# craston/object_detection_cib

Hardware: AMD Instinct MI355X
Metric: images/sec YOLOv5s 640px train (higher is better)
Workload: dtype bf16; 1 GPU; yv5s coco-zipf-like synthetic, 640px, bf16 storage/fp32 accumulate, batch 64/GPU, fwd+assign+loss+bwd+SGD, targets 4-30 boxes/img; global_batch=64, parallelism=dp1, launch=hipGraph replay, collectives=none, launcher=none, attempt=0

## Files before the change

### object_detection_cib_amd/csrc/bn_act.hip

```cpp
#include "kodhip_common.h"
#include <stdlib.h>

namespace {

__device__ __forceinline__ double wave_sum_partials(const float* p, int T, int lane) {
  double a0 = 0.0, a1 = 0.0, a2 = 0.0, a3 = 0.0;
  const int T4 = ((reinterpret_cast<uintptr_t>(p) & 15) == 0) ? (T & ~3) : 0;
#pragma unroll 4
  for (int t = lane * 4; t < T4; t += 256) {
    f32x4 v = *reinterpret_cast<const f32x4*>(p + t);
    a0 += (double)v[0]; a1 += (double)v[1]; a2 += (double)v[2]; a3 += (double)v[3];
  }
  for (int t = T4 + lane; t < T; t += 64) a0 += (double)p[t];
  return wave_sum_d((a0 + a1) + (a2 + a3));
}

__device__ __forceinline__ void wave_sum_partials2(const float* p, const float* q, int T, int lane, double& sp, double& sq) {
  const bool al = ((reinterpret_cast<uintptr_t>(p) | reinterpret_cast<uintptr_t>(q)) & 15) == 0;
  if (!al || T > 4 * 256) {
    sp = wave_sum_partials(p, T, lane);
    sq = wave_sum_partials(q, T, lane);
    return;
  }
  const int T4 = T & ~3;
  const int t0 = lane * 4, t1 = t0 + 256 * 1, t2 = t0 + 256 * 2, t3 = t0 + 256 * 3;
  const f32x4 z = {0.f, 0.f, 0.f, 0.f};
  f32x4 pv[4], qv[4];
  const int ts[4] = {t0, t1, t2, t3};
#pragma unroll
  for (int i = 0; i < 4; ++i) {
    pv[i] = ts[i] < T4 ? *reinterpret_cast<const f32x4*>(p + ts[i]) : z;
    qv[i] = ts[i] < T4 ? *reinterpret_cast<const f32x4*>(q + ts[i]) : z;
  }
  float pt = 0.f, qt = 0.f;
  const bool tail = T4 + lane < T;
  if (tail) { pt = p[T4 + lane]; qt = q[T4 + lane]; }
  double a[4] = {0.0, 0.0, 0.0, 0.0}, b[4] = {0.0, 0.0, 0.0, 0.0};
#pragma unroll
  for (int i = 0; i < 4; ++i) {
    if (ts[i] < T4) {
#pragma unroll
      for (int e = 0; e < 4; ++e) { a[e] += (double)pv[i][e]; b[e] += (double)qv[i][e]; }
    }
  }
  if (tail) { a[0] += (double)pt; b[0] += (double)qt; }
  sp = wave_sum_d((a[0] + a[1]) + (a[2] + a[3]));
  sq = wave_sum_d((b[0] + b[1]) + (b[2] + b[3]));
}

__device__ __forceinline__ void peer_allreduce2(const KodPeerView& pv, unsigned int slot, int idx0, int idx1, int lane,
                                                double& s0, double& s1) {
  const unsigned int seq = *pv.seq;
  const unsigned long long b0 = __shfl((unsigned long long)__double_as_longlong(s0), 0, 64);
  const unsigned long long b1 = __shfl((unsigned long long)__double_as_longlong(s1), 0, 64);
  const int g = lane & 3;
  const unsigned long long gi = (unsigned long long)slot + 2ull * (unsigned long long)(g < 2 ? idx0 : idx1) + (g & 1);
  if (lane < 4) {
    const unsigned long long bits = g < 2 ? b0 : b1;
    const unsigned int payload = (unsigned int)((g & 1) ? (bits >> 32) : bits);
    __hip_atomic_store(pv.peers[pv.rank] + gi, ((unsigned long long)seq << 32) | payload, __ATOMIC_RELAXED, __HIP_MEMORY_SCOPE_SYSTEM);
  }
  unsigned int got = 0;
  bool bad = false;
  const int r = lane >> 2;
  if (r < pv.world) got = (unsigned int)kod_peer_poll(pv, pv.peers[r] + gi, seq, bad);
  double t0 = 0.0, t1 = 0.0;
  for (int q = 0; q < pv.world; ++q) {
    const unsigned long long lo0 = __shfl(got, 4 * q + 0, 64), hi0 = __shfl(got, 4 * q + 1, 64);
    const unsigned long long lo1 = __shfl(got, 4 * q + 2, 64), hi1 = __shfl(got, 4 * q + 3, 64);
    t0 += __longlong_as_double((long long)((hi0 << 32) | lo0));
    t1 += __longlong_as_double((long long)((hi1 << 32) | lo1));
  }
  if (__ballot(bad) != 0ull) t0 = t1 = __longlong_as_double(0x7ff8000000000000ll);
  s0 = t0; s1 = t1;
}

__global__ void bn_reduce_partials_kernel(const float* part, double* sums, int C, int T) {
  int idx = blockIdx.x * (blockDim.x >> 6) + (threadIdx.x >> 6);
  if (idx >= 2 * C) return;
  int lane = threadIdx.x & 63;
  double s = wave_sum_partials(part + (size_t)idx * T, T, lane);
  if (lane == 0) sums[idx] = s;
}

__global__ void bn_finalize_kernel(const double* sums, double count, const float* gamma, const float* beta,
                                   float* running_mean, float* running_var, float momentum, float eps,
                                   float* scale, float* shift, float* mean_out, float* rstd_out, int C,
                                   int update_running) {
  int c = blockIdx.x * blockDim.x + threadIdx.x;
  if (c >= C) return;
  double mean = sums[c] / count;
  double var = sums[C + c] / count - mean * mean;
  if (var < 0.0) var = 0.0;
  float rstd = (float)(1.0 / sqrt(var + (double)eps));
  float g = gamma[c], b = beta[c];
  float sc = g * rstd;
  scale[c] = sc;
  shift[c] = b - (float)mean * sc;
  mean_out[c] = (float)mean;
  rstd_out[c] = rstd;
  if (update_running) {
    double unbiased = count > 1.0 ? var * count / (count - 1.0) : var;
    running_mean[c] = (1.f - momentum) * running_mean[c] + momentum * (float)mean;
    running_var[c] = (1.f - momentum) * running_var[c] + momentum * (float)unbiased;
  }
}

template <bool PEER>
__global__ void bn_finalize_fused_kernel(const float* part, int T, double count, const float* gamma,
                                         const float* beta, float* running_mean, float* running_var,
                                         float momentum, float eps, float* scale, float* shift, float* mean_out,
                                         float* rstd_out, int C, int update_running, KodPeerView pv, unsigned int slot) {
  int c = blockIdx.x * (blockDim.x >> 6) + (threadIdx.x >> 6);
  if (c >= C) return;
  int lane = threadIdx.x & 63;
  const float* p0 = part + (size_t)c * T;
  const float* p1 = part + (size_t)(C + c) * T;
  const float g = gamma[c], b = beta[c];
  const float rm0 = update_running ? running_mean[c] : 0.f, rv0 = update_running ? running_var[c] : 0.f;
  double s0, s1;
  wave_sum_partials2(p0, p1, T, lane, s0, s1);
  if constexpr (PEER) peer_allreduce2(pv, slot, c, C + c, lane, s0, s1);
  if (lane != 0) return;
  double mean = s0 / count;
  double var = s1 / count - mean * mean;
  if (var < 0.0) var = 0.0;
  float rstd = (float)(1.0 / sqrt(var + (double)eps));
  float sc = g * rstd;
  scale[c] = sc;
  shift[c] = b - (float)mean * sc;
  mean_out[c] = (float)mean;
  rstd_out[c] = rstd;
  if (update_running) {
    double unbiased = count > 1.0 ? var * count / (count - 1.0) : var;
    running_mean[c] = (1.f - momentum) * rm0 + momentum * (float)mean;
    running_var[c] = (1.f - momentum) * rv0 + momentum * (float)unbiased;
  }
}

template <bool PEER = false, bool EVAL = false>
__device__ __forceinline__ void bn_bwd_coeffs_channel(const float* part, int T, double count, const float* gamma,
                                                      const float* mean, const float* rstd, float* dgamma, float* dbeta,
                                                      float* coef, int C, int raw_moment, int c, int lane,
                                                      const KodPeerView* pv = nullptr, unsigned int slot = 0) {
  const float* p0 = part + (size_t)c * T;
  const float* p1 = part + (size_t)(C + c) * T;
  const float g_ = gamma[c], rs_ = rstd[c], mu_ = mean[c];
  double s0, s1;
  wave_sum_partials2(p0, p1, T, lane, s0, s1);
  if (raw_moment) s1 = (double)rs_ * (s1 - (double)mu_ * s0);
  if (lane == 0) {
    dbeta[c] = (float)s0;
    dgamma[c] = (float)s1;
  }
  if constexpr (EVAL) {
    static_assert(!PEER, "an eval-mode unit exchanges nothing");
    if (lane == 0) {
      coef[c] = (float)((double)g_ * (double)rs_);
      coef[C + c] = 0.f;
      coef[2 * C + c] = 0.f;
    }
    return;
  }
  if constexpr (PEER) peer_allreduce2(*pv, slot, c, C + c, lane, s0, s1);
  if (lane != 0) return;
  double g = g_, rs = rs_, mu = mu_;
  double S0 = s0 / count, S1 = s1 / count;
  coef[c] = (float)(g * rs);
  coef[C + c] = (float)(-g * rs * rs * S1);
  coef[2 * C + c] = (float)(-g * rs * S0 + g * rs * rs * mu * S1);
}

__global__ void bn_bwd_coeffs_fused_kernel(const float* part, int T, double count, const float* gamma,
                                           const float* mean, const float* rstd, float* dgamma, float* dbeta,
                                           float* coef, int C, int raw_moment) {
  int c = blockIdx.x * (blockDim.x >> 6) + (threadIdx.x >> 6);
  if (c >= C) return;
  bn_bwd_coeffs_channel(part, T, count, gamma, mean, rstd, dgamma, dbeta, coef, C, raw_moment, c, threadIdx.x & 63);
}

__global__ void bn_bwd_coeffs_peer_kernel(const float* part, int T, double count, const float* gamma,
                                          const float* mean, const float* rstd, float* dgamma, float* dbeta,
                                          float* coef, int C, int raw_moment, KodPeerView pv, unsigned int slot) {
  int c = blockIdx.x * (blockDim.x >> 6) + (threadIdx.x >> 6);
  if (c >= C) return;
  bn_bwd_coeffs_channel<true>(part, T, count, gamma, mean, rstd, dgamma, dbeta, coef, C, raw_moment, c, threadIdx.x & 63, &pv, slot);
}

struct CoefJob { const float* part; int T; double count; const float* gamma; const float* mean; const float* rstd;
                 float* dgamma; float* dbeta; float* coef; int C; int raw_moment; };
__global__ void bn_bwd_coeffs_fused2_kernel(CoefJob j0, CoefJob j1) {
  const CoefJob& j = blockIdx.y == 0 ? j0 : j1;
  int c = blockIdx.x * (blockDim.x >> 6) + (threadIdx.x >> 6);
  if (c >= j.C) return;
  bn_bwd_coeffs_channel(j.part, j.T, j.count, j.gamma, j.mean, j.rstd, j.dgamma, j.dbeta, j.coef, j.C, j.raw_moment, c,
                        threadIdx.x & 63);
}

__global__ void bn_bwd_coeffs_eval_kernel(const float* part, int T, const float* gamma, const float* mean,
                                          const float* rstd, float* dgamma, float* dbeta, float* coef, int C,
                                          int raw_moment) {
  int c = blockIdx.x * (blockDim.x >> 6) + (threadIdx.x >> 6);
  if (c >= C) return;
  bn_bwd_coeffs_channel<false, true>(part, T, 1.0, gamma, mean, rstd, dgamma, dbeta, coef, C, raw_moment, c,
                                     threadIdx.x & 63);
}

__global__ void bn_bwd_coeffs_mode2_kernel(CoefJob j0, CoefJob j1, int eval0, int eval1) {
  const CoefJob& j = blockIdx.y == 0 ? j0 : j1;
  int c = blockIdx.x * (blockDim.x >> 6) + (threadIdx.x >> 6);
  if (c >= j.C) return;
  if (blockIdx.y == 0 ? eval0 : eval1)
    bn_bwd_coeffs_channel<false, true>(j.part, j.T, j.count, j.gamma, j.mean, j.rstd, j.dgamma, j.dbeta, j.coef, j.C,
                                       j.raw_moment, c, threadIdx.x & 63);
  else
    bn_bwd_coeffs_channel(j.part, j.T, j.count, j.gamma, j.mean, j.rstd, j.dgamma, j.dbeta, j.coef, j.C, j.raw_moment,
                          c, threadIdx.x & 63);
}

struct BnEvalDesc {
  const float* gamma; const float* beta; const float* running_mean; const float* running_var;
  float* aff; float* coef; long long C; long long reserved;
};

__global__ __launch_bounds__(256) void bn_eval_constants_kernel(const BnEvalDesc* desc, float eps) {
  const BnEvalDesc d = desc[blockIdx.x];
  const int C = (int)d.C;
  for (int c = threadIdx.x; c < C; c += blockDim.x) {
    const float g = d.gamma[c], b = d.beta[c], rm = d.running_mean[c];
    const float rstd = (float)(1.0 / sqrt((double)d.running_var[c] + (double)eps));
    const float sc = g * rstd;
    d.aff[c] = sc;
    d.aff[C + c] = b - rm * sc;
    d.aff[2 * C + c] = rm;
    d.aff[3 * C + c] = rstd;
    if (d.coef != nullptr) {
      d.coef[c] = (float)((double)g * (double)rstd);
      d.coef[C + c] = 0.f;
      d.coef[2 * C + c] = 0.f;
    }
  }
}

constexpr int U = 4;

template <int ACT, int U, bool LDSK, int MAXT>
__global__ __launch_bounds__(MAXT) void bn_silu_apply_kernel(const bf16_t* y, int ldy, const float* scale, const float* shift,
                                     const bf16_t* res, int ldr, int rcoff,
                                     bf16_t* out, int ldo, int ocoff, long M, int C, int rows_per_block_iter, float slope) {
  extern __shared__ float kconst[];
// ... 488 lines not shown
```

### object_detection_cib_amd/csrc/kodhip_common.h

```cpp
#pragma once
#include <hip/hip_runtime.h>
#include <stdint.h>
#include <stdio.h>
#include <type_traits>

typedef __bf16 bf16_t;
typedef __bf16 bf16x8 __attribute__((ext_vector_type(8)));
typedef __bf16 bf16x4 __attribute__((ext_vector_type(4)));
typedef float f32x16 __attribute__((ext_vector_type(16)));
typedef float f32x4 __attribute__((ext_vector_type(4)));
typedef short s16x4 __attribute__((ext_vector_type(4)));
typedef unsigned int u32x4 __attribute__((ext_vector_type(4)));

#define KOD_OK 0
#define KOD_EARG (-1)

extern "C" void kodhip_set_error(const char* fmt, ...);

#define KOD_CHECK_ARG(cond, ...)                 \
  do {                                           \
    if (!(cond)) {                               \
      kodhip_set_error(__VA_ARGS__);             \
      return KOD_EARG;                           \
    }                                            \
  } while (0)

#define KOD_LAUNCH_CHECK(name)                                             \
  do {                                                                     \
    hipError_t e__ = hipGetLastError();                                    \
    if (e__ != hipSuccess) {                                               \
      kodhip_set_error("%s: %s", name, hipGetErrorString(e__));            \
      return (int)e__;                                                     \
    }                                                                      \
  } while (0)

#ifndef KOD_NO_NT
template <typename V> __device__ __forceinline__ V kod_load_once(const void* p) { return __builtin_nontemporal_load(reinterpret_cast<const V*>(p)); }
#else
template <typename V> __device__ __forceinline__ V kod_load_once(const void* p) { return *reinterpret_cast<const V*>(p); }
#endif

__device__ __forceinline__ float bf2f(bf16_t v) { return (float)v; }
__device__ __forceinline__ bf16_t f2bf(float v) { return (bf16_t)v; }

__device__ __forceinline__ float silu_f(float z) { return z / (1.0f + __expf(-z)); }
__device__ __forceinline__ float sigmoid_f(float z) { return 1.0f / (1.0f + __expf(-z)); }

#define KOD_NEG_LOG2E (-1.4426950408889634f)
__device__ __forceinline__ float kod_sigmoid_l2(float zl) {
  return __builtin_amdgcn_rcpf(1.0f + __builtin_amdgcn_exp2f(zl));
}
__device__ __forceinline__ float kod_silu_bwd(float g, float z, float sg) {
  const float t = __builtin_fmaf(-z, sg, z);
  return g * __builtin_fmaf(sg, t, sg);
}

enum { ACT_SILU = 0, ACT_RELU = 1, ACT_LEAKY = 2, ACT_HARDSWISH = 3, ACT_IDENTITY = 4 };
template <int ACT> __device__ __forceinline__ float kod_act(float z, float slope) {
  if (ACT == ACT_SILU) return z * kod_sigmoid_l2(KOD_NEG_LOG2E * z);
  if (ACT == ACT_RELU) return z > 0.f ? z : 0.f;
  if (ACT == ACT_LEAKY) return z > 0.f ? z : z * slope;
  if (ACT == ACT_HARDSWISH) return z * fminf(fmaxf(z + 3.f, 0.f), 6.f) / 6.f;
  return z;
}
template <int ACT> __device__ __forceinline__ float kod_act_bwd(float g, float z, float slope) {
  if (ACT == ACT_SILU) return kod_silu_bwd(g, z, kod_sigmoid_l2(KOD_NEG_LOG2E * z));
  if (ACT == ACT_RELU) return z > 0.f ? g : 0.f;
  if (ACT == ACT_LEAKY) return z > 0.f ? g : g * slope;
  if (ACT == ACT_HARDSWISH) return z <= -3.f ? 0.f : (z < 3.f ? g * ((z / 3.f) + 0.5f) : g);
  return g;
}
template <bool SILU = true, typename F> __host__ __device__ __forceinline__ void kod_with_act(int act, F&& f) {
  if constexpr (SILU) {
    if (act == ACT_SILU) return f(std::integral_constant<int, ACT_SILU>{});
  }
  if (act == ACT_RELU) f(std::integral_constant<int, ACT_RELU>{});
  else if (act == ACT_LEAKY) f(std::integral_constant<int, ACT_LEAKY>{});
  else if (act == ACT_HARDSWISH) f(std::integral_constant<int, ACT_HARDSWISH>{});
  else f(std::integral_constant<int, ACT_IDENTITY>{});
}

__device__ __forceinline__ float wave_sum(float v) {
#pragma unroll
  for (int o = 32; o > 0; o >>= 1) v += __shfl_xor(v, o, 64);
  return v;
}
__device__ __forceinline__ double wave_sum_d(double v) {
#pragma unroll
  for (int o = 32; o > 0; o >>= 1) v += __shfl_xor(v, o, 64);
  return v;
}

#define KOD_PEER_MAX 8
struct KodPeerView {
  unsigned long long* peers[KOD_PEER_MAX];
  int world, rank;
  const unsigned int* seq;
  int* timeout_flag;
  int* host_flag;
  long max_spins;
};

__device__ __forceinline__ unsigned long long kod_peer_poll(const KodPeerView& pv, const unsigned long long* src,
                                                            unsigned int seq, bool& bad) {
  const int raised = __hip_atomic_load(pv.timeout_flag, __ATOMIC_RELAXED, __HIP_MEMORY_SCOPE_AGENT);
  unsigned long long v = 0;
  long spins = 0;
  for (;;) {
    v = __hip_atomic_load(src, __ATOMIC_RELAXED, __HIP_MEMORY_SCOPE_SYSTEM);
    const unsigned int tag = (unsigned int)(v >> 32);
    if (tag == seq) break;
    int why = 0;
    if ((int)(tag - seq) > 0) why = 2;
    else if (raised) why = raised;
    else if (++spins > pv.max_spins) why = 1;
    if (why) {
      bad = true;
      if (!raised) {
        __hip_atomic_store(pv.timeout_flag, why, __ATOMIC_RELAXED, __HIP_MEMORY_SCOPE_AGENT);
        __hip_atomic_store(pv.host_flag, why, __ATOMIC_RELAXED, __HIP_MEMORY_SCOPE_SYSTEM);
      }
      break;
    }
    __builtin_amdgcn_s_sleep(8);
  }
  return v;
}

static inline int cdiv(long a, long b) { return (int)((a + b - 1) / b); }
static inline uint32_t magic_u32(uint32_t d) { return (uint32_t)(((1ull << 32) + d - 1) / d); }
```

### object_detection_cib_amd/csrc/misc_ops.hip

```cpp
#include "kodhip_common.h"

namespace {

__global__ void nchw_to_nhwc4_kernel(const float* x, bf16_t* y, int B, int C, long HW) {
  long i = (long)blockIdx.x * blockDim.x + threadIdx.x;
  if (i >= (long)B * HW) return;
  long b = i / HW, p = i - b * HW;
  bf16x4 v;
#pragma unroll
  for (int c = 0; c < 4; ++c) v[c] = (bf16_t)(c < C ? x[(b * C + c) * HW + p] : 0.f);
  *reinterpret_cast<bf16x4*>(y + i * 4) = v;
}

__global__ void nchw_to_nhwc4_x4_kernel(const float* x, bf16_t* y, int B, int C, long HW) {
  const long q = (long)blockIdx.x * blockDim.x + threadIdx.x;
  const long HWq = HW >> 2;
  if (q >= (long)B * HWq) return;
  const long b = q / HWq, pq = q - b * HWq;
  f32x4 pl[4];
#pragma unroll
  for (int c = 0; c < 4; ++c)
    pl[c] = c < C ? kod_load_once<f32x4>(x + (b * C + c) * HW + pq * 4) : f32x4{0.f, 0.f, 0.f, 0.f};
  bf16x8 o0, o1;
  const float* f0 = reinterpret_cast<const float*>(&pl[0]);
// ... 109 lines not shown
    const bf16_t* row = xb + (long)ry[r] * W * ldx;
#pragma unroll
    for (int c = 0; c < 8; ++c) dst[c] = *reinterpret_cast<const uint2*>(row + (long)cx[c] * ldx);
  };
  load_row(0, cur);
#pragma unroll
  for (int r = 0; r < 8; ++r) {
    if (r + 1 < 8) load_row(r + 1, nxt);
#pragma unroll
    for (int e = 0; e < 4; ++e) {
      uint32_t k[8];
#pragma unroll
      for (int c = 0; c < 8; ++c) {
        const uint32_t d = (e < 2) ? cur[c].x : cur[c].y;
        const uint32_t xf = (e & 1) ? (d & 0xffff0000u) : (d << 16);
        k[c] = pool_key(xf, (uint32_t)(127 - (r * 16 + c))) & cmask[c];
      }
      uint32_t o4[4];
      pool_max5of8(k, o4);
#pragma unroll
      for (int o = 0; o < 4; ++o) hm[r][o][e] = o4[o] & rmask[r];
    }
#pragma unroll
    for (int c = 0; c < 8; ++c) cur[c] = nxt[c];
  }
#pragma unroll
  for (int o = 0; o < 4; ++o) {
    uint32_t best[4][4];
#pragma unroll
    for (int e = 0; e < 4; ++e) {
      uint32_t k[8], o4[4];
#pragma unroll
      for (int r = 0; r < 8; ++r) k[r] = hm[r][o][e];
      pool_max5of8(k, o4);
#pragma unroll
      for (int q = 0; q < 4; ++q) best[q][e] = o4[q];
    }
    if (ox0 + o >= W) continue;
#pragma unroll
    for (int q = 0; q < 4; ++q) {
      if (oy0 + q >= H) continue;
      uint32_t hv[4], ib = 0;
#pragma unroll
      for (int e = 0; e < 4; ++e) {
        const uint32_t K = best[q][e];
        const uint32_t t = (uint32_t)((int32_t)K >> 31) & 0x7fffffffu;
        hv[e] = ~(K ^ t);
        ib |= ((uint32_t)(127 - (q * 16 + o)) - (K & 127u)) << (8 * e);
      }
      const long op = (long)(b * H + oy0 + q) * W + ox0 + o;
      uint2 v;
      v.x = (hv[0] >> 16) | (hv[1] & 0xffff0000u);
      v.y = (hv[2] >> 16) | (hv[3] & 0xffff0000u);
      *reinterpret_cast<uint2*>(y + op * ldy + ycoff + c4 * 4) = v;
      *reinterpret_cast<uint32_t*>(idx + op * C + c4 * 4) = ib;
    }
  }
}

__global__ __launch_bounds__(256) void maxpool5_fwd_kernel(const bf16_t* x, int ldx, int xcoff, bf16_t* y, int ldy, int ycoff,
                                    unsigned char* idx, int B, int H, int W, int C) {
  const int C4 = C >> 2;
  const int WG = (W + 3) >> 2, HG = (H + 3) >> 2;
  long i = (long)blockIdx.x * blockDim.x + threadIdx.x;
  const long total = (long)B * HG * WG * C4;
  if (i >= total) return;
  const int c4 = (int)(i % C4);
  long p = i / C4;
  const int gx = (int)(p % WG);
  p /= WG;
  const int gy = (int)(p % HG);
  const int b = (int)(p / HG);
  maxpool5_fwd_body(x, ldx, xcoff, y, ldy, ycoff, idx, H, W, C, b, gy, gx, c4);
}

constexpr int POOL_BWD_THREADS = 128;
template <int POOL_BWD_THREADS>
__device__ __forceinline__ void maxpool5_bwd_body(float* w0, float* w1, float* w2, float* w3,
                                                  const bf16_t* dy, int ldy, int ycoff, const unsigned char* idx,
                                                  bf16_t* dx, int ldx, int xcoff, int H, int W, int C, const float* dx32,
                                                  int b, int gy, int gx, int c4) {
  const int ix0 = gx * 4, iy0 = gy * 4;
  float* const mine4[4] = {w0, w1, w2, w3};
#pragma unroll
  for (int ri = 0; ri < 4; ++ri)
#pragma unroll
    for (int ci = 0; ci < 4; ++ci) {
      const bool in = iy0 + ri < H && ix0 + ci < W;
      const long po = ((long)(b * H + (in ? iy0 + ri : 0)) * W + (in ? ix0 + ci : 0)) * ldx + xcoff + c4 * 4;
      uint2 old = {0u, 0u};
      if (in && !dx32) old = *reinterpret_cast<const uint2*>(dx + po);
#pragma unroll
      for (int e = 0; e < 4; ++e) {
        const uint32_t d = e < 2 ? old.x : old.y;
        mine4[e][(ri * 4 + ci) * POOL_BWD_THREADS] =
            in ? (dx32 ? dx32[po + e] : __uint_as_float((e & 1) ? (d & 0xffff0000u) : (d << 16))) : 0.f;
      }
    }
  uint32_t ck[8], rk[8];
  int coff_i[8], coff_g[8];
  long roff[8];
#pragma unroll
  for (int c = 0; c < 8; ++c) {
    const int ox = ix0 - 2 + c, oy = iy0 - 2 + c;
    ck[c] = (uint32_t)c + ((ox >= 0 && ox < W) ? 0u : 0x1000u);
    rk[c] = (uint32_t)(16 * c - 0x44) + ((oy >= 0 && oy < H) ? 0u : 0x1000u);
    const int cxc = ox < 0 ? 0 : (ox >= W ? W - 1 : ox), ryc = oy < 0 ? 0 : (oy >= H ? H - 1 : oy);
    coff_i[c] = cxc * C;
    coff_g[c] = cxc * ldy;
    roff[c] = (long)(b * H + ryc) * W;
  }
  const unsigned char* ibase = idx + c4 * 4;
  const bf16_t* gbase = dy + ycoff + c4 * 4;
  uint32_t ibc[8], ibn[8];
  uint2 gc[8], gn[8];
  auto load_row = [&](const int r, uint32_t (&ib)[8], uint2 (&g)[8]) {
    const unsigned char* ir = ibase + roff[r] * C;
    const bf16_t* gr = gbase + roff[r] * ldy;
#pragma unroll
    for (int c = 0; c < 8; ++c) {
      ib[c] = *reinterpret_cast<const uint32_t*>(ir + coff_i[c]);
      g[c] = *reinterpret_cast<const uint2*>(gr + coff_g[c]);
    }
  };
  load_row(7, ibc, gc);
#pragma unroll
  for (int r = 7; r >= 0; --r) {
    if (r > 0) load_row(r - 1, ibn, gn);
#pragma unroll
    for (int c = 0; c < 8; ++c) {
      uint32_t word[4];
      float g[4], cur[4];
#pragma unroll
      for (int e = 0; e < 4; ++e) {
        const uint32_t t = ((ibc[c] >> (8 * e)) & 0xffu) + rk[r] + ck[c];
        const uint32_t pos = ((t >> 2) & 12u) | (t & 3u);
        word[e] = (t & ~0x33u) == 0u ? pos : 16u;
        const uint32_t d = e < 2 ? gc[c].x : gc[c].y;
        g[e] = __uint_as_float((e & 1) ? (d & 0xffff0000u) : (d << 16));
      }
#pragma unroll
      for (int e = 0; e < 4; ++e) cur[e] = mine4[e][word[e] * POOL_BWD_THREADS];
#pragma unroll
      for (int e = 0; e < 4; ++e) mine4[e][word[e] * POOL_BWD_THREADS] = cur[e] + g[e];
    }
#pragma unroll
    for (int c = 0; c < 8; ++c) { ibc[c] = ibn[c]; gc[c] = gn[c]; }
  }
#pragma unroll
  for (int ri = 0; ri < 4; ++ri) {
    if (iy0 + ri >= H) continue;
#pragma unroll
    for (int ci = 0; ci < 4; ++ci) {
      if (ix0 + ci >= W) continue;
      bf16x4 v;
#pragma unroll
      for (int e = 0; e < 4; ++e) v[e] = (bf16_t)mine4[e][(ri * 4 + ci) * POOL_BWD_THREADS];
      *reinterpret_cast<bf16x4*>(dx + ((long)(b * H + iy0 + ri) * W + ix0 + ci) * ldx + xcoff + c4 * 4) = v;
    }
  }
}

__global__ __launch_bounds__(POOL_BWD_THREADS) void maxpool5_bwd_kernel(const bf16_t* dy, int ldy, int ycoff, const unsigned char* idx,
                                    bf16_t* dx, int ldx, int xcoff, int B, int H, int W, int C, const float* dx32) {
  __shared__ float words0[17 * POOL_BWD_THREADS], words1[17 * POOL_BWD_THREADS], words2[17 * POOL_BWD_THREADS], words3[17 * POOL_BWD_THREADS];
  const int C4 = C >> 2;
  const int WG = (W + 3) >> 2, HG = (H + 3) >> 2;
  long i = (long)blockIdx.x * blockDim.x + threadIdx.x;
  const long total = (long)B * HG * WG * C4;
  if (i >= total) return;
  const int c4 = (int)(i % C4);
  long p = i / C4;
  const int gx = (int)(p % WG);
  p /= WG;
  const int gy = (int)(p % HG);
  const int b = (int)(p / HG);
  maxpool5_bwd_body<POOL_BWD_THREADS>(words0 + threadIdx.x, words1 + threadIdx.x, words2 + threadIdx.x, words3 + threadIdx.x,
                                      dy, ldy, ycoff, idx, dx, ldx, xcoff, H, W, C, dx32, b, gy, gx, c4);
}

__global__ __launch_bounds__(256) void maxpool_k_fwd_kernel(const bf16_t* x, int ldx, int xcoff, bf16_t* y, int ldy, int ycoff,
                                                            unsigned char* idx, int B, int H, int W, int C, int K) {
  const int C8 = C >> 3;
  const long i = (long)blockIdx.x * blockDim.x + threadIdx.x;
  if (i >= (long)B * H * W * C8) return;
  const int c8 = (int)(i % C8);
  const long p = i / C8;
  const int ox = (int)(p % W), oy = (int)((p / W) % H), b = (int)(p / ((long)W * H));
  const int r = K >> 1;
  float best[8];
  int tap[8];
  bool first = true;
  for (int dy = 0; dy < K; ++dy) {
    const int iy = oy + dy - r;
    if (iy < 0 || iy >= H) continue;
    for (int dx = 0; dx < K; ++dx) {
      const int ix = ox + dx - r;
      if (ix < 0 || ix >= W) continue;
      const bf16x8 v = *reinterpret_cast<const bf16x8*>(x + ((long)(b * H + iy) * W + ix) * ldx + xcoff + c8 * 8);
#pragma unroll
      for (int e = 0; e < 8; ++e) {
        const float f = (float)v[e];
        if (first) { best[e] = -INFINITY; tap[e] = dy * 16 + dx; }
        if (f > best[e] || f != f) { best[e] = f; tap[e] = dy * 16 + dx; }
      }
      first = false;
    }
  }
  bf16x8 o;
  unsigned long long ib = 0;
#pragma unroll
  for (int e = 0; e < 8; ++e) { o[e] = (bf16_t)best[e]; ib |= (unsigned long long)(tap[e] & 0xff) << (8 * e); }
  *reinterpret_cast<bf16x8*>(y + p * ldy + ycoff + c8 * 8) = o;
  *reinterpret_cast<unsigned long long*>(idx + p * C + c8 * 8) = ib;
}

__global__ __launch_bounds__(256) void maxpool_k_bwd_kernel(const bf16_t* dy, int ldy, int ycoff, const unsigned char* idx,
                                                            bf16_t* dx, int ldx, int xcoff, int B, int H, int W, int C, int K,
                                                            const float* dx32) {
  const int C8 = C >> 3;
  const long i = (long)blockIdx.x * blockDim.x + threadIdx.x;
  if (i >= (long)B * H * W * C8) return;
  const int c8 = (int)(i % C8);
  const long p = i / C8;
  const int ix = (int)(p % W), iy = (int)((p / W) % H), b = (int)(p / ((long)W * H));
  const int r = K >> 1;
  float acc[8];
  bf16_t* d = dx + p * ldx + xcoff + c8 * 8;
  if (dx32) {
#pragma unroll
    for (int e = 0; e < 8; ++e) acc[e] = dx32[p * ldx + xcoff + c8 * 8 + e];
  } else {
    const bf16x8 old = *reinterpret_cast<const bf16x8*>(d);
#pragma unroll
    for (int e = 0; e < 8; ++e) acc[e] = (float)old[e];
  }
  for (int oy = max(iy - r, 0); oy <= min(iy + r, H - 1); ++oy)
    for (int ox = max(ix - r, 0); ox <= min(ix + r, W - 1); ++ox) {
      const long q = (long)(b * H + oy) * W + ox;
      const unsigned long long ib = *reinterpret_cast<const unsigned long long*>(idx + q * C + c8 * 8);
      const bf16x8 g = *reinterpret_cast<const bf16x8*>(dy + q * ldy + ycoff + c8 * 8);
      const unsigned me = (unsigned)((iy - oy + r) * 16 + (ix - ox + r));
#pragma unroll
      for (int e = 0; e < 8; ++e)
        if (((ib >> (8 * e)) & 0xffu) == me) acc[e] += (float)g[e];
    }
  bf16x8 o;
#pragma unroll
  for (int e = 0; e < 8; ++e) o[e] = (bf16_t)acc[e];
  *reinterpret_cast<bf16x8*>(d) = o;
}

__global__ void upsample2x_fwd_kernel(const bf16_t* x, int ldx, int xcoff, bf16_t* y, int ldy, int ycoff,
                                      int B, int H, int W, int C) {
  const int CC = C >> 3;
  long i = (long)blockIdx.x * blockDim.x + threadIdx.x;
  long total = (long)B * 4 * H * W * CC;
  if (i >= total) return;
  int cc = (int)(i % CC);
  long p = i / CC;
  int ox = (int)(p % (2 * W));
  long q = p / (2 * W);
  int oy = (int)(q % (2 * H));
  int b = (int)(q / (2 * H));
  bf16x8 v = *reinterpret_cast<const bf16x8*>(x + ((long)(b * H + (oy >> 1)) * W + (ox >> 1)) * ldx + xcoff + cc * 8);
  *reinterpret_cast<bf16x8*>(y + p * ldy + ycoff + cc * 8) = v;
}

__global__ void upsample2x_bwd_kernel(const bf16_t* dy, int ldy, int ycoff, bf16_t* dx, int ldx, int xcoff,
                                      int accumulate, int B, int H, int W, int C, const float* dx32) {
  const int CC = C >> 3;
  long i = (long)blockIdx.x * blockDim.x + threadIdx.x;
  long total = (long)B * H * W * CC;
  if (i >= total) return;
  int cc = (int)(i % CC);
  long p = i / CC;
  int ix = (int)(p % W);
  long q = p / W;
  int iy = (int)(q % H);
  int b = (int)(q / H);
  float acc[8];
  bf16_t* d = dx + p * ldx + xcoff + cc * 8;
  if (accumulate && dx32) {
    const float* o32 = dx32 + p * ldx + xcoff + cc * 8;
#pragma unroll
    for (int e = 0; e < 8; ++e) acc[e] = o32[e];
  } else if (accumulate) {
    bf16x8 old = *reinterpret_cast<const bf16x8*>(d);
#pragma unroll
    for (int e = 0; e < 8; ++e) acc[e] = (float)old[e];
  } else {
#pragma unroll
    for (int e = 0; e < 8; ++e) acc[e] = 0.f;
  }
#pragma unroll
  for (int s = 0; s < 4; ++s) {
    long op = (long)(b * 2 * H + 2 * iy + (s >> 1)) * (2 * W) + 2 * ix + (s & 1);
    bf16x8 g = *reinterpret_cast<const bf16x8*>(dy + op * ldy + ycoff + cc * 8);
#pragma unroll
    for (int e = 0; e < 8; ++e) acc[e] += (float)g[e];
  }
  bf16x8 o;
#pragma unroll
  for (int e = 0; e < 8; ++e) o[e] = (bf16_t)acc[e];
  *reinterpret_cast<bf16x8*>(d) = o;
}

__global__ __launch_bounds__(256) void head_bwd_prep_kernel(const float* g, bf16_t* dy, float* bpart, int B, int HW,
                                                            int A, int nc, int Npad, uint32_t magic_p, int PREP_ROWS) {
  extern __shared__ float sm[];
  const int P = 5 + nc;
  const int N = A * P;
  const int ldt = Npad + 1;
  const long M = (long)B * HW;
  const int ntiles = (int)((M + PREP_ROWS - 1) / PREP_ROWS);
  float bsum = 0.f;
  for (int i = threadIdx.x; i < PREP_ROWS * ldt; i += blockDim.x) sm[i] = 0.f;
  __syncthreads();
  for (int t = blockIdx.x; t < ntiles; t += gridDim.x) {
    const long m0 = (long)t * PREP_ROWS;
    const int b0 = (int)(m0 / HW), pix0 = (int)(m0 - (long)b0 * HW);
    constexpr int UNR = 4;
    const int per_an = PREP_ROWS * P;
    for (int an = 0; an < A; ++an)
      for (int base = 0; base < per_an; base += UNR * blockDim.x) {
        float v[UNR];
        int dst[UNR];
#pragma unroll
        for (int u = 0; u < UNR; ++u) {
          const int idx = base + u * blockDim.x + threadIdx.x;
          v[u] = 0.f; dst[u] = -1;
          if (idx < per_an) {
            const int r = (int)__umulhi((uint32_t)idx, magic_p);
            const int slot = idx - r * P;
            if (m0 + r < M) {
              int b = b0, pix = pix0 + r;
              while (pix >= HW) { pix -= HW; ++b; }
              v[u] = g[(((long)b * A + an) * HW + pix) * P + slot];
            }
            dst[u] = r * ldt + (slot < 4 ? 4 * an + slot : (slot == 4 ? 4 * A + an : 5 * A + an * nc + slot - 5));
          }
        }
#pragma unroll
        for (int u = 0; u < UNR; ++u)
          if (dst[u] >= 0) sm[dst[u]] = v[u];
      }
    __syncthreads();
    const int cpr = Npad / 8;
    for (int c = threadIdx.x; c < PREP_ROWS * cpr; c += blockDim.x) {
// ... 213 lines not shown
}

__global__ void stamp_kernel(unsigned long long* dst) { *dst = wall_clock64(); }

__global__ __launch_bounds__(256) void pull_host_kernel(const uint4* __restrict__ src, uint4* __restrict__ dst, long n16) {
  for (long i = (long)blockIdx.x * blockDim.x + threadIdx.x; i < n16; i += (long)gridDim.x * blockDim.x) dst[i] = src[i];
}

}

extern "C" {

int kodhip_nchw_to_nhwc4(const float* x, void* y, int B, int C, int H, int W, hipStream_t stream) {
  KOD_CHECK_ARG(x && y && B > 0 && C > 0 && C <= 4 && H > 0 && W > 0, "nchw_to_nhwc4: bad args");
  long n = (long)B * H * W;
  if (((long)H * W) % 4 == 0 && ((uintptr_t)x % 16) == 0)
    hipLaunchKernelGGL(nchw_to_nhwc4_x4_kernel, dim3(cdiv(n / 4, 256)), dim3(256), 0, stream, x, (bf16_t*)y, B, C, (long)H * W);
  else
    hipLaunchKernelGGL(nchw_to_nhwc4_kernel, dim3(cdiv(n, 256)), dim3(256), 0, stream, x, (bf16_t*)y, B, C, (long)H * W);
  KOD_LAUNCH_CHECK("nchw_to_nhwc4");
  return KOD_OK;
}

int kodhip_pack_weights(const float* master, void* fpack, void* dpack, const void* descs, int nlayers,
                        long total_blocks, hipStream_t stream) {
  KOD_CHECK_ARG(master && fpack && descs && nlayers > 0 && total_blocks > 0, "pack_weights: bad args");
  hipLaunchKernelGGL(pack_weights_kernel, dim3((unsigned)total_blocks), dim3(256), 0, stream, master, (bf16_t*)fpack,
                     (bf16_t*)dpack, (const PackDesc*)descs, nlayers);
  KOD_LAUNCH_CHECK("pack_weights");
  return KOD_OK;
}
int kodhip_pack_desc_bytes(void) { return (int)sizeof(PackDesc); }

int kodhip_maxpool5_fwd(const void* x, int ldx, int xcoff, void* y, int ldy, int ycoff, void* idx,
                        int B, int H, int W, int C, hipStream_t stream) {
  KOD_CHECK_ARG(x && y && idx && C % 8 == 0 && ldx % 8 == 0 && ldy % 8 == 0 && xcoff % 8 == 0 && ycoff % 8 == 0,
                "maxpool5_fwd: bad args");
  long n = (long)B * ((H + 3) / 4) * ((W + 3) / 4) * (C / 4);
  hipLaunchKernelGGL(maxpool5_fwd_kernel, dim3(cdiv(n, 256)), dim3(256), 0, stream, (const bf16_t*)x, ldx, xcoff,
                     (bf16_t*)y, ldy, ycoff, (unsigned char*)idx, B, H, W, C);
  KOD_LAUNCH_CHECK("maxpool5_fwd");
  return KOD_OK;
}

int kodhip_maxpool5_bwd(const void* dy, int ldy, int ycoff, const void* idx, void* dx, int ldx, int xcoff,
                        int B, int H, int W, int C, const float* dx_f32, hipStream_t stream) {
  KOD_CHECK_ARG(dy && dx && idx && C % 8 == 0 && ldx % 8 == 0 && ldy % 8 == 0 && xcoff % 8 == 0 && ycoff % 8 == 0,
                "maxpool5_bwd: bad args");
  long n = (long)B * ((H + 3) / 4) * ((W + 3) / 4) * (C / 4);
  hipLaunchKernelGGL(maxpool5_bwd_kernel, dim3(cdiv(n, POOL_BWD_THREADS)), dim3(POOL_BWD_THREADS), 0, stream, (const bf16_t*)dy, ldy, ycoff,
                     (const unsigned char*)idx, (bf16_t*)dx, ldx, xcoff, B, H, W, C, dx_f32);
  KOD_LAUNCH_CHECK("maxpool5_bwd");
  return KOD_OK;
}

int kodhip_maxpool_fwd(const void* x, int ldx, int xcoff, void* y, int ldy, int ycoff, void* idx,
                       int B, int H, int W, int C, int K, hipStream_t stream) {
  if (K == 5) return kodhip_maxpool5_fwd(x, ldx, xcoff, y, ldy, ycoff, idx, B, H, W, C, stream);
  KOD_CHECK_ARG(x && y && idx && C % 8 == 0 && ldx % 8 == 0 && ldy % 8 == 0 && xcoff % 8 == 0 && ycoff % 8 == 0, "maxpool_fwd: bad args");
  KOD_CHECK_ARG(K >= 1 && K <= 15 && (K & 1), "maxpool_fwd: window %d (odd sizes up to 15)", K);
  const long n = (long)B * H * W * (C / 8);
  hipLaunchKernelGGL(maxpool_k_fwd_kernel, dim3(cdiv(n, 256)), dim3(256), 0, stream, (const bf16_t*)x, ldx, xcoff, (bf16_t*)y, ldy, ycoff,
                     (unsigned char*)idx, B, H, W, C, K);
  KOD_LAUNCH_CHECK("maxpool_fwd");
  return KOD_OK;
}

int kodhip_maxpool_bwd(const void* dy, int ldy, int ycoff, const void* idx, void* dx, int ldx, int xcoff,
                       int B, int H, int W, int C, int K, const float* dx_f32, hipStream_t stream) {
  if (K == 5) return kodhip_maxpool5_bwd(dy, ldy, ycoff, idx, dx, ldx, xcoff, B, H, W, C, dx_f32, stream);
  KOD_CHECK_ARG(dy && dx && idx && C % 8 == 0 && ldx % 8 == 0 && ldy % 8 == 0 && xcoff % 8 == 0 && ycoff % 8 == 0, "maxpool_bwd: bad args");
  KOD_CHECK_ARG(K >= 1 && K <= 15 && (K & 1), "maxpool_bwd: window %d (odd sizes up to 15)", K);
  const long n = (long)B * H * W * (C / 8);
  hipLaunchKernelGGL(maxpool_k_bwd_kernel, dim3(cdiv(n, 256)), dim3(256), 0, stream, (const bf16_t*)dy, ldy, ycoff, (const unsigned char*)idx,
                     (bf16_t*)dx, ldx, xcoff, B, H, W, C, K, dx_f32);
  KOD_LAUNCH_CHECK("maxpool_bwd");
  return KOD_OK;
}

int kodhip_upsample2x_fwd(const void* x, int ldx, int xcoff, void* y, int ldy, int ycoff,
                          int B, int H, int W, int C, hipStream_t stream) {
  KOD_CHECK_ARG(x && y && C % 8 == 0 && ldx % 8 == 0 && ldy % 8 == 0 && xcoff % 8 == 0 && ycoff % 8 == 0,
                "upsample2x_fwd: bad args");
  long n = (long)B * 4 * H * W * (C / 8);
  hipLaunchKernelGGL(upsample2x_fwd_kernel, dim3(cdiv(n, 256)), dim3(256), 0, stream, (const bf16_t*)x, ldx, xcoff,
                     (bf16_t*)y, ldy, ycoff, B, H, W, C);
  KOD_LAUNCH_CHECK("upsample2x_fwd");
  return KOD_OK;
}

int kodhip_upsample2x_bwd(const void* dy, int ldy, int ycoff, void* dx, int ldx, int xcoff, int accumulate,
                          int B, int H, int W, int C, const float* dx_f32, hipStream_t stream) {
  KOD_CHECK_ARG(dy && dx && C % 8 == 0 && ldx % 8 == 0 && ldy % 8 == 0 && xcoff % 8 == 0 && ycoff % 8 == 0,
                "upsample2x_bwd: bad args");
  long n = (long)B * H * W * (C / 8);
  hipLaunchKernelGGL(upsample2x_bwd_kernel, dim3(cdiv(n, 256)), dim3(256), 0, stream, (const bf16_t*)dy, ldy, ycoff,
                     (bf16_t*)dx, ldx, xcoff, accumulate, B, H, W, C, dx_f32);
  KOD_LAUNCH_CHECK("upsample2x_bwd");
  return KOD_OK;
}

int kodhip_head_bwd_prep(const float* g, void* dy, float* workspace, float* db_box, float* db_obj, float* db_cls,
                         int B, int HW, int A, int nc, int Npad, hipStream_t stream) {
  KOD_CHECK_ARG(g && dy && workspace && db_box && db_obj && db_cls, "head_bwd_prep: null pointer");
  KOD_CHECK_ARG(Npad % 8 == 0 && Npad >= A * (5 + nc) && Npad <= 256, "head_bwd_prep: bad Npad");
  KOD_CHECK_ARG(nc > 0 && 5 + nc <= 128, "head_bwd_prep: bad class count");
  long M = (long)B * HW;
  const int PREP_ROWS = Npad <= 128 ? 64 : 32;
  int grid = (int)((M + PREP_ROWS - 1) / PREP_ROWS);
  if (grid > 2048) grid = 2048;
  hipLaunchKernelGGL(head_bwd_prep_kernel, dim3(grid), dim3(256), PREP_ROWS * (Npad + 1) * sizeof(float), stream, g,
                     (bf16_t*)dy, workspace, B, HW, A, nc, Npad, magic_u32((uint32_t)(5 + nc)), PREP_ROWS);
  KOD_LAUNCH_CHECK("head_bwd_prep");
  hipLaunchKernelGGL(head_bias_reduce_kernel, dim3(cdiv(A * (5 + nc), 4)), dim3(256), 0, stream,
                     (const float*)workspace, grid, Npad, db_box, db_obj, db_cls, A, nc);
  KOD_LAUNCH_CHECK("head_bias_reduce");
  return KOD_OK;
}

int kodhip_sgd_nesterov(float* params, const float* grads, float* momentum_buf, const void* group_ids,
                        long n, const float* hyper, hipStream_t stream) {
  KOD_CHECK_ARG(params && grads && momentum_buf && group_ids && hyper && n > 0 && n % 64 == 0, "sgd_nesterov: bad args");
  hipLaunchKernelGGL(sgd_nesterov_kernel, dim3(cdiv(n / 4, 256)), dim3(256), 0, stream, params, grads, momentum_buf,
                     (const unsigned char*)group_ids, n, hyper);
  KOD_LAUNCH_CHECK("sgd_nesterov");
  return KOD_OK;
}

int kodhip_sgd_nesterov_masked(float* params, const float* grads, float* momentum_buf, const void* group_ids,
                               const void* keep_mask, long n, const float* hyper, hipStream_t stream) {
  KOD_CHECK_ARG(params && grads && momentum_buf && group_ids && keep_mask && hyper && n > 0 && n % 64 == 0,
                "sgd_nesterov_masked: bad args");
  hipLaunchKernelGGL(sgd_nesterov_masked_kernel, dim3(cdiv(n / 4, 256)), dim3(256), 0, stream, params, grads, momentum_buf,
                     (const unsigned char*)group_ids, (const unsigned char*)keep_mask, n, hyper);
  KOD_LAUNCH_CHECK("sgd_nesterov_masked");
  return KOD_OK;
}

int kodhip_clip_block_bytes(void) { return KOD_CLIP_FLOATS * (int)sizeof(float); }
int kodhip_grad_norm_workspace_bytes(void) { return KOD_NORM_BLOCKS * 3 * (int)sizeof(double); }

int kodhip_grad_norm(const float* grads, const void* group_ids, const void* count_mask, long n, const float* hyper,
                     float* clip, void* workspace, int skip_nonfinite, int nontemporal, hipStream_t stream) {
  KOD_CHECK_ARG(grads && group_ids && hyper && clip && workspace && n > 0 && n % 64 == 0 && ((uintptr_t)workspace % 8) == 0,
                "grad_norm: bad args");
  int grid = cdiv(n / 4, 256);
  if (grid > KOD_NORM_BLOCKS) grid = KOD_NORM_BLOCKS;
  if (nontemporal)
    hipLaunchKernelGGL(grad_norm_partial_kernel<true>, dim3(grid), dim3(256), 0, stream, grads, (const unsigned char*)group_ids,
                       (const unsigned char*)count_mask, n, hyper, (double*)workspace);
  else
    hipLaunchKernelGGL(grad_norm_partial_kernel<false>, dim3(grid), dim3(256), 0, stream, grads, (const unsigned char*)group_ids,
                       (const unsigned char*)count_mask, n, hyper, (double*)workspace);
  KOD_LAUNCH_CHECK("grad_norm");
  hipLaunchKernelGGL(grad_norm_finalize_kernel, dim3(1), dim3(64), 0, stream, (const double*)workspace, grid, clip, skip_nonfinite);
  KOD_LAUNCH_CHECK("grad_norm_finalize");
  return KOD_OK;
}

int kodhip_sgd_nesterov_clipped(float* params, const float* grads, float* momentum_buf, const void* group_ids,
                                const void* keep_mask, long n, const float* hyper, const float* clip, int mode,
                                int skip_nonfinite, hipStream_t stream) {
  KOD_CHECK_ARG(params && grads && momentum_buf && group_ids && hyper && clip && n > 0 && n % 64 == 0,
                "sgd_nesterov_clipped: bad args");
  KOD_CHECK_ARG(mode == KOD_CLIP_NORM || mode == KOD_CLIP_VALUE, "sgd_nesterov_clipped: unknown mode %d", mode);
  const dim3 grid(cdiv(n / 4, 256)), blk(256);
  const unsigned char* gid = (const unsigned char*)group_ids;
// ... 57 lines not shown
```

Baseline: 5513 images/sec.

## Use DPP/permlane wave reductions, restructure pool backward loads, and upsample per input pixel

Replaces the shuffle-based double wave reductions in BN finalize and backward-coefficient kernels with permlane swap and DPP sequences, and reduces the two sums jointly so their latency chains interleave. The two divisions by count are also computed in parallel lanes and exchanged with one DPP move. The maxpool backward kernel now issues all 16 old-gradient loads up front and keeps every row of index and gradient data in registers instead of double-buffering, at the cost of more register pressure. Upsample forward now launches one thread per input pixel that writes four outputs, cutting index arithmetic and redundant reads. Ablation macros that stub out loads and reductions are added but are off by default.

```diff
diff --git a/object_detection_cib_amd/csrc/bn_act.hip b/object_detection_cib_amd/csrc/bn_act.hip
--- a/object_detection_cib_amd/csrc/bn_act.hip
+++ b/object_detection_cib_amd/csrc/bn_act.hip
@@ -12,7 +12,7 @@
     a0 += (double)v[0]; a1 += (double)v[1]; a2 += (double)v[2]; a3 += (double)v[3];
   }
   for (int t = T4 + lane; t < T; t += 64) a0 += (double)p[t];
-  return wave_sum_d((a0 + a1) + (a2 + a3));
+  return wave_sum_d_dpp((a0 + a1) + (a2 + a3));
 }
 
 __device__ __forceinline__ void wave_sum_partials2(const float* p, const float* q, int T, int lane, double& sp, double& sq) {
@@ -27,6 +27,14 @@
   const f32x4 z = {0.f, 0.f, 0.f, 0.f};
   f32x4 pv[4], qv[4];
   const int ts[4] = {t0, t1, t2, t3};
+#ifdef KOD_ABL_LAT_NOLOADS
+  const f32x4 lv = {(float)lane, 1.f, 2.f, 3.f};
+#pragma unroll
+  for (int i = 0; i < 4; ++i) { pv[i] = ts[i] < T4 ? lv : z; qv[i] = ts[i] < T4 ? lv : z; }
+  float pt = 0.f, qt = 0.f;
+  const bool tail = T4 + lane < T;
+  if (tail) { pt = (float)lane; qt = (float)lane; }
+#else
 #pragma unroll
   for (int i = 0; i < 4; ++i) {
     pv[i] = ts[i] < T4 ? *reinterpret_cast<const f32x4*>(p + ts[i]) : z;
@@ -35,6 +43,7 @@
   float pt = 0.f, qt = 0.f;
   const bool tail = T4 + lane < T;
   if (tail) { pt = p[T4 + lane]; qt = q[T4 + lane]; }
+#endif
   double a[4] = {0.0, 0.0, 0.0, 0.0}, b[4] = {0.0, 0.0, 0.0, 0.0};
 #pragma unroll
   for (int i = 0; i < 4; ++i) {
@@ -44,8 +53,9 @@
     }
   }
   if (tail) { a[0] += (double)pt; b[0] += (double)qt; }
-  sp = wave_sum_d((a[0] + a[1]) + (a[2] + a[3]));
-  sq = wave_sum_d((b[0] + b[1]) + (b[2] + b[3]));
+  sp = (a[0] + a[1]) + (a[2] + a[3]);
+  sq = (b[0] + b[1]) + (b[2] + b[3]);
+  wave_sum_d2_dpp(sp, sq);
 }
 
 __device__ __forceinline__ void peer_allreduce2(const KodPeerView& pv, unsigned int slot, int idx0, int idx1, int lane,
@@ -121,9 +131,15 @@
   double s0, s1;
   wave_sum_partials2(p0, p1, T, lane, s0, s1);
   if constexpr (PEER) peer_allreduce2(pv, slot, c, C + c, lane, s0, s1);
+#ifdef KOD_ABL_LAT_NOTAIL
+  if (lane == 0) { scale[c] = (float)s0 * g; shift[c] = (float)s1 + b; mean_out[c] = (float)s0 + rm0; rstd_out[c] = (float)s1 + rv0; }
+  return;
+#endif
+  const double quo = (lane == 0 ? s0 : s1) / count;
+  const double quo_n = kod_dpp_d<0xb1>(quo);
   if (lane != 0) return;
-  double mean = s0 / count;
-  double var = s1 / count - mean * mean;
+  double mean = quo;
+  double var = quo_n - mean * mean;
   if (var < 0.0) var = 0.0;
   float rstd = (float)(1.0 / sqrt(var + (double)eps));
   float sc = g * rstd;
@@ -163,9 +179,15 @@
     return;
   }
   if constexpr (PEER) peer_allreduce2(*pv, slot, c, C + c, lane, s0, s1);
+#ifdef KOD_ABL_LAT_NOTAIL
+  if (lane == 0) { coef[c] = (float)s0 * g_; coef[C + c] = (float)s1 * rs_; coef[2 * C + c] = (float)s0 + mu_; }
+  return;
+#endif
+  const double quo = (lane == 0 ? s0 : s1) / count;
+  const double quo_n = kod_dpp_d<0xb1>(quo);
   if (lane != 0) return;
   double g = g_, rs = rs_, mu = mu_;
-  double S0 = s0 / count, S1 = s1 / count;
+  double S0 = quo, S1 = quo_n;
   coef[c] = (float)(g * rs);
   coef[C + c] = (float)(-g * rs * rs * S1);
   coef[2 * C + c] = (float)(-g * rs * S0 + g * rs * rs * mu * S1);
diff --git a/object_detection_cib_amd/csrc/kodhip_common.h b/object_detection_cib_amd/csrc/kodhip_common.h
--- a/object_detection_cib_amd/csrc/kodhip_common.h
+++ b/object_detection_cib_amd/csrc/kodhip_common.h
@@ -91,6 +91,37 @@
   return v;
 }
 
+template <int CTRL> __device__ __forceinline__ double kod_dpp_d(double v) {
+  const unsigned long long b = (unsigned long long)__double_as_longlong(v);
+  const unsigned int lo = (unsigned int)__builtin_amdgcn_update_dpp(0, (int)(unsigned int)b, CTRL, 0xf, 0xf, true);
+  const unsigned int hi = (unsigned int)__builtin_amdgcn_update_dpp(0, (int)(unsigned int)(b >> 32), CTRL, 0xf, 0xf, true);
+  return __longlong_as_double((long long)(((unsigned long long)hi << 32) | lo));
+}
+template <int HALF> __device__ __forceinline__ double kod_swap_pair_sum_d(double v) {
+  const unsigned long long b = (unsigned long long)__double_as_longlong(v);
+  const unsigned int lo = (unsigned int)b, hi = (unsigned int)(b >> 32);
+  const auto rl = HALF == 32 ? __builtin_amdgcn_permlane32_swap(lo, lo, false, false) : __builtin_amdgcn_permlane16_swap(lo, lo, false, false);
+  const auto rh = HALF == 32 ? __builtin_amdgcn_permlane32_swap(hi, hi, false, false) : __builtin_amdgcn_permlane16_swap(hi, hi, false, false);
+  return __longlong_as_double((long long)(((unsigned long long)rh[0] << 32) | rl[0])) +
+         __longlong_as_double((long long)(((unsigned long long)rh[1] << 32) | rl[1]));
+}
+__device__ __forceinline__ void wave_sum_d2_dpp(double& a, double& b) {
+#ifdef KOD_ABL_LAT_NORED
+  return;
+#endif
+  a = kod_swap_pair_sum_d<32>(a); b = kod_swap_pair_sum_d<32>(b);
+  a = kod_swap_pair_sum_d<16>(a); b = kod_swap_pair_sum_d<16>(b);
+  a += kod_dpp_d<0x128>(a); b += kod_dpp_d<0x128>(b);
+  a += kod_dpp_d<0x141>(kod_dpp_d<0x1b>(a)); b += kod_dpp_d<0x141>(kod_dpp_d<0x1b>(b));
+  a += kod_dpp_d<0x4e>(a); b += kod_dpp_d<0x4e>(b);
+  a += kod_dpp_d<0xb1>(a); b += kod_dpp_d<0xb1>(b);
+}
+__device__ __forceinline__ double wave_sum_d_dpp(double v) {
+  double unused = 0.0;
+  wave_sum_d2_dpp(v, unused);
+  return v;
+}
+
 #define KOD_PEER_MAX 8
 struct KodPeerView {
   unsigned long long* peers[KOD_PEER_MAX];
diff --git a/object_detection_cib_amd/csrc/misc_ops.hip b/object_detection_cib_amd/csrc/misc_ops.hip
--- a/object_detection_cib_amd/csrc/misc_ops.hip
+++ b/object_detection_cib_amd/csrc/misc_ops.hip
@@ -215,20 +215,38 @@
                                                   int b, int gy, int gx, int c4) {
   const int ix0 = gx * 4, iy0 = gy * 4;
   float* const mine4[4] = {w0, w1, w2, w3};
+  float old[16][4];
+  long po[16];
+#pragma unroll
+  for (int i = 0; i < 16; ++i) {
+    const int ri = i >> 2, ci = i & 3;
+    const bool in = iy0 + ri < H && ix0 + ci < W;
+    po[i] = ((long)(b * H + (in ? iy0 + ri : 0)) * W + (in ? ix0 + ci : 0)) * ldx + xcoff + c4 * 4;
+  }
+  if (dx32) {
+#pragma unroll
+    for (int i = 0; i < 16; ++i)
+#pragma unroll
+      for (int e = 0; e < 4; ++e) old[i][e] = dx32[po[i] + e];
+  } else {
+    uint2 o2[16];
+#pragma unroll
+    for (int i = 0; i < 16; ++i) o2[i] = *reinterpret_cast<const uint2*>(dx + po[i]);
+#pragma unroll
+    for (int i = 0; i < 16; ++i)
+#pragma unroll
+      for (int e = 0; e < 4; ++e) {
+        const uint32_t d = e < 2 ? o2[i].x : o2[i].y;
+        old[i][e] = __uint_as_float((e & 1) ? (d & 0xffff0000u) : (d << 16));
+      }
+  }
 #pragma unroll
   for (int ri = 0; ri < 4; ++ri)
 #pragma unroll
     for (int ci = 0; ci < 4; ++ci) {
       const bool in = iy0 + ri < H && ix0 + ci < W;
-      const long po = ((long)(b * H + (in ? iy0 + ri : 0)) * W + (in ? ix0 + ci : 0)) * ldx + xcoff + c4 * 4;
-      uint2 old = {0u, 0u};
-      if (in && !dx32) old = *reinterpret_cast<const uint2*>(dx + po);
-#pragma unroll
-      for (int e = 0; e < 4; ++e) {
-        const uint32_t d = e < 2 ? old.x : old.y;
-        mine4[e][(ri * 4 + ci) * POOL_BWD_THREADS] =
-            in ? (dx32 ? dx32[po + e] : __uint_as_float((e & 1) ? (d & 0xffff0000u) : (d << 16))) : 0.f;
-      }
+#pragma unroll
+      for (int e = 0; e < 4; ++e) mine4[e][(ri * 4 + ci) * POOL_BWD_THREADS] = in ? old[ri * 4 + ci][e] : 0.f;
     }
   uint32_t ck[8], rk[8];
   int coff_i[8], coff_g[8];
@@ -245,8 +263,8 @@
   }
   const unsigned char* ibase = idx + c4 * 4;
   const bf16_t* gbase = dy + ycoff + c4 * 4;
-  uint32_t ibc[8], ibn[8];
-  uint2 gc[8], gn[8];
+  uint32_t iball[8][8];
+  uint2 gall[8][8];
   auto load_row = [&](const int r, uint32_t (&ib)[8], uint2 (&g)[8]) {
     const unsigned char* ir = ibase + roff[r] * C;
     const bf16_t* gr = gbase + roff[r] * ldy;
@@ -256,10 +274,12 @@
       g[c] = *reinterpret_cast<const uint2*>(gr + coff_g[c]);
     }
   };
-  load_row(7, ibc, gc);
+  load_row(7, iball[7], gall[7]);
 #pragma unroll
   for (int r = 7; r >= 0; --r) {
-    if (r > 0) load_row(r - 1, ibn, gn);
+    if (r > 0) load_row(r - 1, iball[r - 1], gall[r - 1]);
+    const uint32_t (&ibc)[8] = iball[r];
+    const uint2 (&gc)[8] = gall[r];
 #pragma unroll
     for (int c = 0; c < 8; ++c) {
       uint32_t word[4];
@@ -277,8 +297,6 @@
 #pragma unroll
       for (int e = 0; e < 4; ++e) mine4[e][word[e] * POOL_BWD_THREADS] = cur[e] + g[e];
     }
-#pragma unroll
-    for (int c = 0; c < 8; ++c) { ibc[c] = ibn[c]; gc[c] = gn[c]; }
   }
 #pragma unroll
   for (int ri = 0; ri < 4; ++ri) {
@@ -388,16 +406,21 @@
                                       int B, int H, int W, int C) {
   const int CC = C >> 3;
   long i = (long)blockIdx.x * blockDim.x + threadIdx.x;
-  long total = (long)B * 4 * H * W * CC;
+  long total = (long)B * H * W * CC;
   if (i >= total) return;
   int cc = (int)(i % CC);
   long p = i / CC;
-  int ox = (int)(p % (2 * W));
-  long q = p / (2 * W);
-  int oy = (int)(q % (2 * H));
-  int b = (int)(q / (2 * H));
-  bf16x8 v = *reinterpret_cast<const bf16x8*>(x + ((long)(b * H + (oy >> 1)) * W + (ox >> 1)) * ldx + xcoff + cc * 8);
-  *reinterpret_cast<bf16x8*>(y + p * ldy + ycoff + cc * 8) = v;
+  int ix = (int)(p % W);
+  long q = p / W;
+  int iy = (int)(q % H);
+  int b = (int)(q / H);
+  const bf16x8 v = *reinterpret_cast<const bf16x8*>(x + p * ldx + xcoff + cc * 8);
+  bf16_t* o = y + (((long)(b * 2 * H + 2 * iy)) * (2 * W) + 2 * ix) * ldy + ycoff + cc * 8;
+  const long row = (long)(2 * W) * ldy;
+  *reinterpret_cast<bf16x8*>(o) = v;
+  *reinterpret_cast<bf16x8*>(o + ldy) = v;
+  *reinterpret_cast<bf16x8*>(o + row) = v;
+  *reinterpret_cast<bf16x8*>(o + row + ldy) = v;
 }
 
 __global__ void upsample2x_bwd_kernel(const bf16_t* dy, int ldy, int ycoff, bf16_t* dx, int ldx, int xcoff,
@@ -777,7 +800,7 @@
                           int B, int H, int W, int C, hipStream_t stream) {
   KOD_CHECK_ARG(x && y && C % 8 == 0 && ldx % 8 == 0 && ldy % 8 == 0 && xcoff % 8 == 0 && ycoff % 8 == 0,
                 "upsample2x_fwd: bad args");
-  long n = (long)B * 4 * H * W * (C / 8);
+  long n = (long)B * H * W * (C / 8);
   hipLaunchKernelGGL(upsample2x_fwd_kernel, dim3(cdiv(n, 256)), dim3(256), 0, stream, (const bf16_t*)x, ldx, xcoff,
                      (bf16_t*)y, ldy, ycoff, B, H, W, C);
   KOD_LAUNCH_CHECK("upsample2x_fwd");
```

Measured after the change: 5536 images/sec (median of 6 runs). Within noise of the previous version (+0.4%).
